# OpenNLPLab/ACR_WSSS

Hardware: AMD Instinct MI355X
Metric: img/s ACR-ViT-hybrid-base 448x448 train step (higher is better)
Workload: dtype f32_split; 1 GPU; BASELINE configs[1]: ViT-hybrid-base (DPT) 448x448, batch 16 per GPU, ACR train step (2 views, fwd+bwd+SGD); global_batch=16, classes=20, alpha=125, parallelism=dp1

## Files before the change

### acr_wsss_amd/_lib.py

```python
import ctypes
import os

import torch

_HERE = os.path.dirname(os.path.abspath(__file__))
LIB_PATH = os.environ.get("ACR_LIB_PATH") or os.path.join(_HERE, "libacr_hip.so")

ACR_F32, ACR_BF16, ACR_BF16_F32MATH, ACR_F32_BF16X3 = 0, 1, 2, 3
MATH = {"f32": 0, "f32_split": 1, "f32_fp16x2": 2}
BF16_F32MATH = False
GETAM_FUNCS = {"grad": 0, "cam_grad": 1, "grad_s": 2, "cam_grad_s": 3}

c_void_p, c_int32, c_int64, c_float, c_size_t = (ctypes.c_void_p, ctypes.c_int32, ctypes.c_int64,
                                                  ctypes.c_float, ctypes.c_size_t)


class AttnDesc(ctypes.Structure):
    _fields_ = [("B", c_int32), ("H", c_int32), ("T", c_int32), ("head_dim", c_int32),
                ("dtype", c_int32), ("scale", c_float),
                ("qkv_sb", c_int64), ("qkv_st", c_int64), ("qkv_sh", c_int64),
                ("o_sb", c_int64), ("o_st", c_int64), ("o_sh", c_int64)]


_P = ctypes.POINTER(AttnDesc)
# ... 3 lines not shown
    "acr_set_option": (c_int32, [c_int32, c_int32]),
    "acr_get_option": (c_int32, [c_int32]),
    "acr_attn_fwd": (c_int32, [_P, c_void_p, c_void_p, c_void_p, c_void_p, c_void_p, c_void_p, c_int64, c_int64,
                               c_void_p]),
    "acr_attn_bwd": (c_int32, [_P, c_void_p, c_void_p, c_void_p, c_void_p, c_void_p, c_void_p, c_void_p, c_int64,
                               c_int64, c_void_p, c_void_p, c_void_p, c_void_p, c_void_p]),
    "acr_attn_scores_floats": (c_int64, [_P]),
    "acr_attn_fwd_scores": (c_int32, [_P, c_void_p, c_void_p, c_void_p, c_void_p, c_void_p, c_void_p, c_void_p, c_int64, c_int64,
                                      c_void_p]),
    "acr_attn_fwd_scores_oimg": (c_int32, [_P, c_void_p, c_void_p, c_void_p, c_void_p, c_void_p, c_void_p, c_void_p, c_int64, c_int64,
                                           c_void_p, c_void_p]),
    "acr_attn_fwd_oimg_offered": (c_int32, [_P]),
    "acr_attn_bwd_scores": (c_int32, [_P, c_void_p, c_void_p, c_void_p, c_void_p, c_void_p, c_void_p, c_void_p, c_void_p, c_int64,
                                      c_int64, c_void_p, c_void_p, c_void_p, c_void_p, c_void_p]),
    "acr_attn_bwd_ws_floats": (c_int64, [_P]),
    "acr_split3_bf16": (c_int32, [c_void_p, c_int64, c_int64, c_int64, c_void_p, c_int64, c_void_p]),
    "acr_attn_probs": (c_int32, [_P, c_void_p, c_void_p, c_void_p, c_void_p, c_void_p]),
    "acr_attn_dprobs": (c_int32, [_P, c_void_p, c_void_p, c_void_p, c_void_p]),
    "acr_consistency_ws_floats": (c_size_t, [c_int32, c_int32, c_int32]),
    "acr_consistency_fwd": (c_int32, [c_void_p, c_void_p, c_int64, c_int32, c_int32, c_int32, c_int32, c_void_p,
                                      c_void_p, c_void_p]),
    "acr_consistency_bwd": (c_int32, [c_void_p, c_void_p, c_int64, c_int32, c_int32, c_int32, c_int32, c_void_p,
                                      c_void_p, c_void_p, c_int64, c_int64, c_void_p]),
    "acr_linear_bf16": (c_int32, [c_void_p, c_int64, c_void_p, c_int64, c_void_p, c_void_p, c_int64, c_void_p, c_int64,
                                  c_int32, c_int32, c_int32, c_void_p]),
    "acr_gemm_f32_ws_floats": (c_size_t, [c_int32, c_int32, c_int32, c_int32, c_int32]),
    "acr_x3_image_floats": (c_size_t, [c_int32, c_int32]),
    "acr_x3_colsum_ws_floats": (c_size_t, [c_int32, c_int32]),
    "acr_x3_image": (c_int32, [c_void_p, c_int64, c_int32, c_int32, c_void_p, c_void_p, c_void_p, c_void_p]),
    "acr_x3_image_t": (c_int32, [c_void_p, c_int64, c_int32, c_int32, c_void_p, c_void_p]),
# ... 184 lines not shown
```

### acr_wsss_amd/csrc/attn_f32.h

```cpp
#pragma once
#include <hip/hip_runtime.h>
#include <stdint.h>

struct AttnGeom {
    int B, H, T;
    float scale;
    int64_t sb, st, sh;
    int64_t osb, ost, osh;
};

void acr_attn_fwd_f32_dma(const AttnGeom& g, const float* q, const float* k, const float* v, float* o, float* lse2, float* pmean,
                          int64_t pmean_sb, int64_t pmean_st, hipStream_t st);
void acr_attn_bwd_f32_dma(const AttnGeom& g, const float* q, const float* k, const float* v, const float* o, const float* d_o,
                          const float* lse2, const float* gm, int64_t gm_sb, int64_t gm_st, float* dq, float* dk, float* dv,
                          float* delta, hipStream_t st);

void acr_attn_fwd_f32_sres(const AttnGeom& g, const float* q, const float* k, const float* v, float* o, float* lse2, float* scores,
                           float* pmean, int64_t pmean_sb, int64_t pmean_st, hipStream_t st);
void acr_attn_bwd_f32_sres(const AttnGeom& g, const float* q, const float* k, const float* v, const float* o, const float* d_o,
                           const float* lse2, const float* scores, const float* gm, int64_t gm_sb, int64_t gm_st, float* dq,
                           float* dk, float* dv, float* delta, hipStream_t st);
void acr_attn_pmean_sres(const AttnGeom& g, const float* scores, const float* lse2, float* pmean, int64_t pmean_sb, int64_t pmean_st,
                         hipStream_t st);
void acr_attn_delta_sres(const AttnGeom& g, const float* scores, const float* o, const float* d_o, const float* lse2, const float* gm,
                         int64_t gm_sb, int64_t gm_st, float* delta, hipStream_t st);

int64_t acr_attn_x3_scores_floats(const AttnGeom& g);
int64_t acr_attn_x3_bwd_ws_floats(const AttnGeom& g);
bool acr_attn_x3_fwd_uses_split_tail(int T);
void acr_attn_fwd_f32_x3(const AttnGeom& g, const float* q, const float* k, const float* v, float* o, float* lse2, float* scores,
                         float* pmean, int64_t pmean_sb, int64_t pmean_st, hipStream_t st, char* oimg = nullptr);
void acr_attn_bwd_f32_x3(const AttnGeom& g, const float* q, const float* k, const float* v, const float* o, const float* d_o,
                         const float* lse2, const float* scores, const float* gm, int64_t gm_sb, int64_t gm_st, float* dq, float* dk,
                         float* dv, float* delta_ws, hipStream_t st);
```

### acr_wsss_amd/csrc/attn_f32.hip

```cpp
#include "acr_common.h"
#include "attn_f32.h"

#define LDP 68
#define TILE_FLOATS (32 * LDP)

template <typename T, int NTHREADS>
__device__ __forceinline__ void stage_tile(float* lds, const T* g, int64_t st, int row0, int Tn, int tid, float mul) {
#pragma unroll
    for (int i = 0; i < 512 / NTHREADS; ++i) {
        const int slot = tid + i * NTHREADS;
        const int row = slot >> 4, c4 = slot & 15;
        f32x4 v = acr_load4<T>(g + (int64_t)min(row0 + row, Tn - 1) * st + c4 * 4) * mul;
        const f32x4 z = {0.f, 0.f, 0.f, 0.f};
        *reinterpret_cast<f32x4*>(lds + row * LDP + c4 * 4) = (row0 + row < Tn) ? v : z;
    }
}

template <typename T>
__device__ __forceinline__ void load_rows(float (&reg)[32], const T* g, int64_t st, int row0, int Tn, int lane, float mul) {
    const int r = lane & 31, h = lane >> 5;
    const float okm = (row0 + r < Tn) ? mul : 0.f;
    const T* p = g + (int64_t)min(row0 + r, Tn - 1) * st + 32 * h;
#pragma unroll
    for (int i = 0; i < 8; ++i) {
// ... 602 lines not shown
                  "acr_attn_fwd_scores_oimg: pmean row pitch < T or batch stride < T*pitch");
    ACR_CHECK_ARG(d->o_sh == 64 && d->o_st == (int64_t)d->H * 64 && d->o_sb == (int64_t)d->T * d->o_st,
                  "acr_attn_fwd_scores_oimg: o must be the dense (B, T, H*64) activation (its image is that of the (B*T) x (H*64) matrix)");
    rc = check_x3(d, "acr_attn_fwd_scores_oimg");
    if (rc) return rc;
    acr_attn_fwd_f32_x3(geom(d), (const float*)q, (const float*)k, (const float*)v, (float*)o, lse2, scores, pmean, pmean_sb, pmean_st,
                        (hipStream_t)stream, reinterpret_cast<char*>(o_image));
    return acr_check_launch("acr_attn_fwd_scores_oimg");
}

extern "C" int acr_attn_fwd_oimg_offered(const acr_attn_desc* d) {
    if (!d || d->dtype != ACR_F32_BF16X3 || d->T <= 0) return 0;
    return acr_attn_x3_fwd_uses_split_tail(d->T) ? 0 : 1;
}

extern "C" int acr_attn_bwd_scores(const acr_attn_desc* d, const void* q, const void* k, const void* v, const void* o,
                                   const void* d_o, const float* lse2, const float* scores, const float* gmean, int64_t gmean_sb,
                                   int64_t gmean_st, void* dq, void* dk, void* dv, float* delta_ws, void* stream) {
    int rc = check_desc(d, "acr_attn_bwd_scores");
    if (rc) return rc;
    if (d->dtype != ACR_F32 && d->dtype != ACR_F32_BF16X3) {
        acr_set_error("acr_attn_bwd_scores: fp32 tensors only (the bf16 kernels recompute the logits)");
        return ACR_ERR_UNSUPPORTED;
    }
    ACR_CHECK_ARG(q && k && v && o && d_o && lse2 && scores && dq && dk && dv && delta_ws, "acr_attn_bwd_scores: null pointer");
    ACR_CHECK_ARG(aligned16(q) && aligned16(k) && aligned16(v) && aligned16(o) && aligned16(d_o) && aligned16(scores),
                  "acr_attn_bwd_scores: inputs must be 16-byte aligned");
    ACR_CHECK_ARG(!gmean || (gmean_st >= d->T && gmean_sb >= (int64_t)d->T * gmean_st),
                  "acr_attn_bwd_scores: gmean row pitch < T or batch stride < T*pitch");
    ACR_CHECK_ARG(!gmean || ((gmean_st & 3) == 0 && (gmean_sb & 3) == 0 && aligned16(gmean)),
                  "acr_attn_bwd_scores: gmean must be 16-byte aligned with pitch and batch stride multiples of 4 floats");
    if (d->dtype == ACR_F32_BF16X3) {
        rc = check_x3(d, "acr_attn_bwd_scores");
        if (rc) return rc;
        ACR_CHECK_ARG(aligned16(delta_ws) && aligned16(dq) && aligned16(dk) && aligned16(dv), "acr_attn_bwd_scores: delta_ws / dq / dk / dv must be 16-byte aligned");
        acr_attn_bwd_f32_x3(geom(d), (const float*)q, (const float*)k, (const float*)v, (const float*)o, (const float*)d_o, lse2, scores,
                            gmean, gmean_sb, gmean_st, (float*)dq, (float*)dk, (float*)dv, delta_ws, (hipStream_t)stream);
        return acr_check_launch("acr_attn_bwd_scores");
    }
    acr_attn_bwd_f32_sres(geom(d), (const float*)q, (const float*)k, (const float*)v, (const float*)o, (const float*)d_o, lse2,
                          scores, gmean, gmean_sb, gmean_st, (float*)dq, (float*)dk, (float*)dv, delta_ws, (hipStream_t)stream);
    return acr_check_launch("acr_attn_bwd_scores");
}

extern "C" int acr_attn_probs(const acr_attn_desc* d, const void* q, const void* k, const float* lse2, float* probs,
                              void* stream) {
    int rc = check_desc(d, "acr_attn_probs");
    if (rc) return rc;
    ACR_CHECK_ARG(q && k && lse2 && probs, "acr_attn_probs: null pointer");
    AttnGeom g = geom(d);
    const int nt = (d->T + 63) / 64;
    ACR_CHECK_ARG((int64_t)d->B * d->H * nt * nt < (1ll << 31), "acr_attn_probs: grid too large");
    const dim3 grid(d->B * d->H * nt * nt);
    const void* pp[2] = {q, k};
    if (d->dtype == ACR_F32)
        hipLaunchKernelGGL((attn_tile_qk_kernel<float, TQK_PROBS>), grid, dim3(256), 0, (hipStream_t)stream, g,
                           (const float*)q, (const float*)k, lse2, probs, (int64_t)0, (int64_t)0);
// ... 66 lines not shown
```

### acr_wsss_amd/csrc/attn_f32_sres_tails.h

```cpp
#pragma once
#include "acr_common.h"
#include "attn_f32.h"
#include "attn_f32_tiles.h"

#define SB_FLOATS 1024
#define SRES_LOAD_NT(p) __builtin_nontemporal_load(reinterpret_cast<const f32x4*>(p))
#define SRES_LOAD(p) (*reinterpret_cast<const f32x4*>(p))
#define SRES_STORE(p, v) __builtin_nontemporal_store(v, reinterpret_cast<f32x4*>(p))
#define SRES_LOAD_DQ(p) SRES_LOAD_NT(p)
#define SRES_DMA_AUX 0

__device__ __forceinline__ int64_t sres_block(const AttnGeom& g, int NB, int b, int hd, int qb, int kb) {
    return ((((int64_t)b * g.H + hd) * NB + qb) * NB + kb) * SB_FLOATS;
}

__device__ __forceinline__ void wave_wait_dma() { asm volatile("s_waitcnt vmcnt(0)" ::: "memory"); }
__device__ __forceinline__ void wave_wait_lds() { asm volatile("s_waitcnt lgkmcnt(0)" ::: "memory"); }

template <int NW>
__device__ __forceinline__ void attn_fwd_tail_body(float* smem, float* mlsh, const AttnGeom& g, const float* __restrict__ q,
                                                   const float* __restrict__ k, const float* __restrict__ v, float* __restrict__ o,
                                                   float* __restrict__ lse2, float* __restrict__ sres, int id) {
    const int NB = (g.T + 31) >> 5;
    const int hd = id % g.H, b = id / g.H;
// ... 159 lines not shown
        const float* pw = smem + w * DT_FLOATS;
#pragma unroll
        for (int e = 0; e < 16; ++e) { dq0[e] += pw[e * 64 + lane]; dq1[e] += pw[(16 + e) * 64 + lane]; }
    }
#pragma unroll
    for (int reg = 0; reg < 16; ++reg) {
        const int qq = q0 + acr_krow(reg, h);
        if (qq < g.T) {
            float* p = dq + base + (int64_t)qq * g.st;
            p[r] = dq0[reg] * g.scale;
            p[32 + r] = dq1[reg] * g.scale;
        }
    }
}

template <int NW>
__device__ __forceinline__ void attn_dkdv_tail_body(float* smem, float* ssm, const AttnGeom& g, const float* __restrict__ q,
                                                    const float* __restrict__ v, const float* __restrict__ d_o,
                                                    const float* __restrict__ lse2, const float* __restrict__ delta,
                                                    const float* __restrict__ sres, const float* __restrict__ gm, int64_t gm_sb,
                                                    int64_t gm_st, float* __restrict__ dk, float* __restrict__ dv, int id) {
    const int NB = (g.T + 31) >> 5;
    const int hd = id % g.H, b = id / g.H;
    const int tid = threadIdx.x, lane = tid & 63;
    const int wave = __builtin_amdgcn_readfirstlane(tid >> 6);
    const int r = lane & 31, h = lane >> 5;
    const int key0 = (NB - 1) * 32;
    const int64_t base = (int64_t)b * g.sb + (int64_t)hd * g.sh;
    const int64_t obase = (int64_t)b * g.osb + (int64_t)hd * g.osh;
    const float* qb = q + base;
    const float* dob = d_o + obase;
    const float* lrow = lse2 + ((int64_t)b * g.H + hd) * g.T;
    const float* drow = delta + ((int64_t)b * g.H + hd) * g.T;
    const float* scol = sres + sres_block(g, NB, b, hd, 0, NB - 1);
    const int64_t sstep = (int64_t)NB * SB_FLOATS;
    float* tl = smem + wave * DT_FLOATS;
// ... 42 lines not shown
                if (q0 + acr_krow(reg, h) >= g.T) s[reg] = -INFINITY;
        }
        f32x16 p, ds;
#pragma unroll
        for (int gq = 0; gq < 4; ++gq) {
            const f32x4 l4 = *reinterpret_cast<const f32x4*>(rcw + 8 * gq + 4 * h);
            const f32x4 d4 = *reinterpret_cast<const f32x4*>(rcw + 32 + 8 * gq + 4 * h);
#pragma unroll
            for (int e = 0; e < 4; ++e) {
                const int reg = 4 * gq + e;
                const float pv = __builtin_amdgcn_exp2f(s[reg] - l4[e]);
                p[reg] = pv;
                ds[reg] = pv * (dp[reg] + gv[reg] - d4[e]);
            }
        }
        accop_a_i<0, 0>(dv0, p, sm, lb);
        accop_a_i<0, 1>(dv1, p, sm, lb);
        wave_wait_lds();
        dma_tile32_one(tl, qb, g.st, q0, g.T, lane);
        wave_wait_dma();
        accop_a_i<0, 0>(dk0, ds, sm, lb);
        accop_a_i<0, 1>(dk1, ds, sm, lb);
        wave_wait_lds();
    }
    __syncthreads();
#pragma unroll
    for (int e = 0; e < 16; ++e) {
        tl[e * 64 + lane] = dk0[e]; tl[(16 + e) * 64 + lane] = dk1[e];
        sw[e * 64 + lane] = dv0[e]; sw[(16 + e) * 64 + lane] = dv1[e];
    }
// ... 27 lines not shown
```

### acr_wsss_amd/csrc/attn_f32_x3.hip

```cpp
#include <type_traits>

#include "acr_split.h"
#include "attn_f32.h"
#include "attn_f32_sres_tails.h"

typedef __bf16 bf16_t;
typedef __attribute__((address_space(3))) void* x3_lds_vp;
typedef const __attribute__((address_space(1))) void* x3_glb_vp;

#define X3_PLANE_B (32 * 64 * 2)
#define X3_TILE_B (3 * X3_PLANE_B)
#define X3_SLOT_B (2 * X3_TILE_B)
#define X3_SB_FLOATS 1024

#define X3_STORE_NT(p, v) __builtin_nontemporal_store(v, reinterpret_cast<f32x4*>(p))
#define X3_LOAD_NT(p) __builtin_nontemporal_load(reinterpret_cast<const f32x4*>(p))


template <int N>
__device__ __forceinline__ void x3_vmcnt() { asm volatile("s_waitcnt vmcnt(%0)" ::"n"(N) : "memory"); }
__device__ __forceinline__ void x3_wait_vm(int n) {
    if (n >= 9) x3_vmcnt<9>();
    else if (n >= 8) x3_vmcnt<8>();
    else if (n >= 7) x3_vmcnt<7>();
// ... 449 lines not shown
        if (k0 + 32 < g.T) step(k0 + 32, std::integral_constant<int, 1>{});
    }
    if (!live) return;
    const int64_t base = (int64_t)b * g.sb + (int64_t)hd * g.sh;
#pragma unroll
    for (int reg = 0; reg < 16; ++reg) {
        const int qq = q0 + acr_krow(reg, h);
        if (qq < g.T) {
            float* p = dq + base + (int64_t)qq * g.st;
            p[r] = dq0[reg] * g.scale;
            p[32 + r] = dq1[reg] * g.scale;
        }
    }
}

__device__ __forceinline__ void attn_dkdv_x3_body(char* smem, float* ssm, float* gsm, float* rcm, int bid, int nblk, bool tails,
                                                  const X3Geom& g,
                                                  const bf16_t* __restrict__ qp, const bf16_t* __restrict__ vp,
                                                  const bf16_t* __restrict__ dop, const float* __restrict__ lse2,
                                                  const float* __restrict__ delta, const float* __restrict__ sres,
                                                  const float* __restrict__ gm, int64_t gm_sb, int64_t gm_st, float* __restrict__ dk,
                                                  float* __restrict__ dv) {
    const int NB = (g.T + 31) >> 5, nkt = tails ? NB / X3_BW : (NB + X3_BW - 1) / X3_BW;
    int id = acr_xcd_remap(bid, nblk);
    const int ktile = id % nkt; id /= nkt;
    const int hd = id % g.H;
    const int b = id / g.H;
    const int tid = threadIdx.x, lane = tid & 63;
    const int wave = __builtin_amdgcn_readfirstlane(tid >> 6);
    const int r = lane & 31, h = lane >> 5;
    const int key0 = (ktile * X3_BW + wave) * 32;
    const bool live = key0 < g.T;
    const int64_t pbase = (int64_t)b * g.T * g.D + (int64_t)hd * 64;
    const int op = wave >> 2, pc = wave & 3;
    const bf16_t* tb = (op ? dop : qp) + pbase;
    char* tdst = smem + op * X3_TILE_B;
    const float* lrow = lse2 + ((int64_t)b * g.H + hd) * g.T;
// ... 39 lines not shown
    f32x16 dk0 = {0}, dk1 = {0}, dv0 = {0}, dv1 = {0};
    const X3Lane lb = x3_lane(lane, smem);
    const int doff = x3_dma_off(g.D, pc, lane);
    uint32_t tb4[4];
    {
        const int gk = r >> 3, hk = (r >> 2) & 1, ek = r & 3, mm = 2 * gk + hk;
#pragma unroll
        for (int j = 0; j < 4; ++j)
            tb4[j] = x3_lds_addr(ssm) + ((wave * 2 * X3_SB_FLOATS) + gk * 256 + 128 * hk + ek + 4 * ((j + 4 * h) ^ mm)) * 4;
    }
    const uint32_t gaddr = x3_lds_addr(gsm) + (wave * X3_SB_FLOATS + 4 * h * 32 + r) * 4;
    const uint32_t rcaddr = x3_lds_addr(rcw) + 16 * h;
    auto step = [&](int q0, auto slot_tag) {
        constexpr int SLOT = decltype(slot_tag)::value;
        constexpr int QOFF = SLOT * X3_SLOT_B, DOOFF = QOFF + X3_TILE_B;
        x3_barrier((q0 > 0 && live) ? 1 + (gb0 ? 4 : 0) + (q0 + 32 < g.T ? 4 : 0) : 0);
        auto dma_next = [&] {
            if (q0 + 64 <= g.T) x3_dma_tile_i(tdst + (SLOT ^ 1) * X3_SLOT_B, tb + (int64_t)(q0 + 32) * g.D, g.plane, doff, pc);
            else if (q0 + 32 < g.T) x3_dma_tile(tdst + (SLOT ^ 1) * X3_SLOT_B, tb, g.plane, g.D, q0 + 32, g.T, pc, lane);
            X3_FENCE();
        };
        if (!live) { dma_next(); return; }
        f32x16 dp = {0};
        x3_rowop<DOOFF>(dp, lb, vf, dma_next);
        if (q0 > 0) x3_wait_vm(q0 + 32 < g.T ? 7 : 0);
        float s[16], gv[16];
        f32x4 l4[4], d4[4];
#define X3_RDS(REG) IMG_RD32(s[REG], tb4[(REG) & 3], SLOT * X3_SB_FLOATS * 4 + 128 * ((REG) >> 2))
#define X3_RDG(REG) IMG_RD32(gv[REG], gaddr, 128 * (((REG) & 3) + 8 * ((REG) >> 2)))
        X3_RDS(0); X3_RDS(1); X3_RDS(2); X3_RDS(3); X3_RDS(4); X3_RDS(5); X3_RDS(6); X3_RDS(7);
        X3_RDS(8); X3_RDS(9); X3_RDS(10); X3_RDS(11); X3_RDS(12); X3_RDS(13); X3_RDS(14); X3_RDS(15);
// ... 17 lines not shown
#pragma unroll
            for (int reg = 0; reg < 16; ++reg)
                if (q0 + acr_krow(reg, h) >= g.T) s[reg] = -INFINITY;
        }
        f32x16 p, ds;
#pragma unroll
        for (int gq = 0; gq < 4; ++gq) {
#pragma unroll
            for (int e = 0; e < 4; ++e) {
                const int reg = 4 * gq + e;
                const float pv = __builtin_amdgcn_exp2f(s[reg] - l4[gq][e]);
                p[reg] = pv;
                ds[reg] = pv * (dp[reg] + gv[reg] * invH - d4[gq][e]);
            }
        }
        asm volatile("s_waitcnt lgkmcnt(0)" ::: "memory");
        bf16x8 z0[3], z1[3];
        split3_bf16_acc<0>(p, z0);
        x3_accop<DOOFF, true>(dv0, dv1, z0, z1, lb,
                              [&] { split3_bf16_acc<1>(p, z1); },
                              [&] { if (q0 + 32 < g.T) dma_rc(q0 + 32); X3_FENCE(); },
                              [&] { if (q0 + 32 < g.T) dma_g(q0 + 32); X3_FENCE(); });
        split3_bf16_acc<0>(ds, z0);
        x3_accop<QOFF, true>(dk0, dk1, z0, z1, lb,
                             [&] { split3_bf16_acc<1>(ds, z1); },
                             [&] { if (q0 + 64 < g.T) dma_scores((q0 >> 5) + 2, SLOT); X3_FENCE(); });
    };
    for (int q0 = 0; q0 < g.T; q0 += 64) {
        step(q0, std::integral_constant<int, 0>{});
        if (q0 + 32 < g.T) step(q0 + 32, std::integral_constant<int, 1>{});
// ... 19 lines not shown
                                                                   const float* __restrict__ lse2, const float* __restrict__ delta,
                                                                   const float* __restrict__ sres, const float* __restrict__ gm,
                                                                   int64_t gm_sb, int64_t gm_st, float* __restrict__ dq,
                                                                   float* __restrict__ dk, float* __restrict__ dv,
                                                                   const float* __restrict__ q32, const float* __restrict__ k32,
                                                                   const float* __restrict__ v32, const float* __restrict__ do32,
                                                                   AttnGeom g32, int ntail) {
    __shared__ __attribute__((aligned(1024))) char lds[2 * X3_SLOT_B + X3_BW * 3 * X3_SB_FLOATS * 4 + X3_BW * 256];
    char* smem = lds;
    float* ssm = reinterpret_cast<float*>(lds + 2 * X3_SLOT_B);
    float* gsm = ssm + X3_BW * 2 * X3_SB_FLOATS;
    float* rcm = gsm + X3_BW * X3_SB_FLOATS;
    const int half = ((int)gridDim.x - 2 * ntail) >> 1;
    const int bid = (int)blockIdx.x;
    if (bid < half)
        attn_dkdv_x3_body(smem, ssm, gsm, rcm, bid, half, ntail != 0, g, qp, vp, dop, lse2, delta, sres, gm, gm_sb, gm_st, dk, dv);
    else if (bid < 2 * half)
        attn_dq_x3_body(smem, ssm, gsm, bid - half, half, ntail != 0, g, kp, vp, dop, lse2, delta, sres, gm, gm_sb, gm_st, dq);
    else if (bid < 2 * half + ntail)
        attn_dkdv_tail_body<X3_BW>(reinterpret_cast<float*>(lds), reinterpret_cast<float*>(lds) + X3_BW * DT_FLOATS, g32, q32, v32, do32, lse2,
                                   delta, sres, gm, gm_sb, gm_st, dk, dv, acr_xcd_remap(bid - 2 * half, ntail));
    else
        attn_dq_tail_body<X3_BW>(reinterpret_cast<float*>(lds), g32, k32, v32, do32, lse2, delta, sres, gm, gm_sb, gm_st, dq,
                                 acr_xcd_remap(bid - 2 * half - ntail, ntail));
}

static int64_t x3_score_floats(const AttnGeom& g) {
    const int64_t nb = (g.T + 31) / 32;
    return (int64_t)g.B * g.H * nb * nb * X3_SB_FLOATS;
}
int64_t acr_attn_x3_scores_floats(const AttnGeom& g) {
    return x3_score_floats(g) + 9 * ((int64_t)g.B * g.T * g.H * 64) / 2;
}
int64_t acr_attn_x3_bwd_ws_floats(const AttnGeom& g) {
    return (((int64_t)g.B * g.H * g.T + 3) & ~(int64_t)3) + 3 * ((int64_t)g.B * g.T * g.H * 64) / 2;
}
static bool x3_split_tail(int NB, int nw) { return (NB % nw) == 1 && NB > nw; }
static X3Geom x3_geom(const AttnGeom& g) {
    X3Geom x;
    x.B = g.B; x.H = g.H; x.T = g.T; x.D = g.H * 64; x.scale = g.scale;
    x.plane = (int64_t)g.B * g.T * x.D;
    x.osb = g.osb; x.ost = g.ost; x.osh = g.osh;
    x.sb = g.sb; x.st = g.st; x.sh = g.sh;
    return x;
}

bool acr_attn_x3_fwd_uses_split_tail(int T) {
    const int NB = (T + 31) / 32;
    return x3_split_tail(NB, 4) && NB >= 33;
}

// ... 3 lines not shown
    bf16_t* planes = reinterpret_cast<bf16_t*>(scores + x3_score_floats(g));
    X3SplitArgs a;
    a.src[0] = q; a.src[1] = k; a.src[2] = v;
    a.sb = g.sb; a.st = g.st; a.sh = g.sh; a.dst = planes; a.plane = x.plane; a.B = g.B; a.T = g.T; a.H = g.H;
    const int64_t n8 = (int64_t)g.B * g.T * g.H * 8;
    hipLaunchKernelGGL(x3_split_kernel, dim3((unsigned)((n8 + 255) / 256), 3), dim3(256), 0, st, a);
    const int NB = (g.T + 31) / 32;
    const int ntail = (acr_attn_x3_fwd_uses_split_tail(g.T) && oimg == nullptr) ? g.B * g.H : 0;
    hipLaunchKernelGGL(attn_fwd_x3_kernel, dim3(g.B * g.H * (ntail ? NB / 4 : (NB + 3) / 4) + ntail), dim3(256), 0, st, x, (const bf16_t*)planes,
                       (const bf16_t*)(planes + 3 * x.plane), (const bf16_t*)(planes + 6 * x.plane), o, lse2, scores, q, k, v, g, ntail, oimg);
    if (pmean) acr_attn_pmean_sres(g, scores, lse2, pmean, pmean_sb, pmean_st, st);
}

void acr_attn_bwd_f32_x3(const AttnGeom& g, const float* q, const float* k, const float* v, const float* o, const float* d_o,
                         const float* lse2, const float* scores, const float* gm, int64_t gm_sb, int64_t gm_st, float* dq, float* dk,
                         float* dv, float* delta_ws, hipStream_t st) {
    const X3Geom x = x3_geom(g);
    const bf16_t* planes = reinterpret_cast<const bf16_t*>(scores + x3_score_floats(g));
    bf16_t* dop = reinterpret_cast<bf16_t*>(delta_ws + (((int64_t)g.B * g.H * g.T + 3) & ~(int64_t)3));
    X3SplitArgs a;
    a.src[0] = d_o; a.src[1] = a.src[2] = nullptr;
    a.sb = g.osb; a.st = g.ost; a.sh = g.osh; a.dst = dop; a.plane = x.plane; a.B = g.B; a.T = g.T; a.H = g.H;
    const int64_t n8 = (int64_t)g.B * g.T * g.H * 8;
    hipLaunchKernelGGL(x3_split_kernel, dim3((unsigned)((n8 + 255) / 256), 1), dim3(256), 0, st, a);
    acr_attn_delta_sres(g, scores, o, d_o, lse2, gm, gm_sb, gm_st, delta_ws, st);
    const int NB = (g.T + 31) / 32;
    const int ntail = x3_split_tail(NB, X3_BW) ? g.B * g.H : 0;
    const int nmain = g.B * g.H * (ntail ? NB / X3_BW : (NB + X3_BW - 1) / X3_BW);
    hipLaunchKernelGGL(attn_bwd_x3_kernel, dim3(2 * nmain + 2 * ntail), dim3(64 * X3_BW), 0, st, x, planes, planes + 3 * x.plane,
                       planes + 6 * x.plane, (const bf16_t*)dop, lse2, (const float*)delta_ws, scores, gm, gm_sb, gm_st, dq, dk, dv, q, k, v, d_o, g,
                       ntail);
}

extern "C" int acr_split3_bf16(const float* x, int64_t rows, int64_t cols, int64_t ld, void* planes, int64_t plane_stride, void* stream) {
    ACR_CHECK_ARG(x && planes, "acr_split3_bf16: null pointer");
    ACR_CHECK_ARG(rows > 0 && cols > 0 && (cols % 8) == 0 && (ld % 4) == 0 && ld >= cols, "acr_split3_bf16: need cols %% 8 == 0, ld %% 4 == 0, ld >= cols");
    ACR_CHECK_ARG(plane_stride >= rows * cols && (plane_stride % 8) == 0, "acr_split3_bf16: plane stride must cover rows * cols and be a multiple of 8");
    ACR_CHECK_ARG(((uintptr_t)x & 15) == 0 && ((uintptr_t)planes & 15) == 0, "acr_split3_bf16: 16-byte alignment");
    const int64_t n = rows * (cols >> 3);
    ACR_CHECK_ARG((n + 255) / 256 < (1ll << 31), "acr_split3_bf16: too large");
    hipLaunchKernelGGL(x3_split2d_kernel, dim3((unsigned)((n + 255) / 256)), dim3(256), 0, (hipStream_t)stream, x, rows, cols, ld,
                       (bf16_t*)planes, plane_stride);
    return acr_check_launch("acr_split3_bf16");
}
```

### acr_wsss_amd/ops.py

```python
import os
import torch
from torch.autograd import Function

from . import _lib as L

HEAD_DIM = 64
ATTN_F32_SCORES = True


def pad4(n):
    return (n + 3) & ~3


def _desc(B, H, T, dtype, packed_qkv=True, math=0):
    D = H * HEAD_DIM
    d = L.AttnDesc()
    d.B, d.H, d.T, d.head_dim = B, H, T, HEAD_DIM
    d.dtype = L.ACR_F32_BF16X3 if (math == 1 and dtype == torch.float32) else L.dtype_code(dtype)
    d.scale = HEAD_DIM ** -0.5
    d.qkv_sb, d.qkv_st, d.qkv_sh = T * 3 * D, 3 * D, HEAD_DIM
    d.o_sb, d.o_st, d.o_sh = T * D, D, HEAD_DIM
    return d


# ... 126 lines not shown
        gm_sb = gm_st = 0
        if g_pm is not None:
            ok = (g_pm.dtype == torch.float32 and g_pm.stride(2) == 1 and g_pm.stride(1) % 4 == 0
                  and g_pm.stride(1) >= pad4(T) and g_pm.stride(0) % 4 == 0 and g_pm.data_ptr() % 16 == 0)
            if not ok:
                buf = torch.zeros((B, T, pad4(T)), dtype=torch.float32, device=qkv.device)
                buf[:, :, :T].copy_(g_pm)
                g_pm = buf[:, :, :T]
            gm_sb, gm_st = g_pm.stride(0), g_pm.stride(1)
        d = _desc(B, heads, T, qkv.dtype, math=ctx.math if scores is not None else 0)
        dqkv = torch.empty_like(qkv)
        delta = torch.empty(lib.acr_attn_bwd_ws_floats(d) if scores is not None else B * heads * T, dtype=torch.float32, device=qkv.device)
        qp, kp, vp = _qkv_ptrs(qkv, heads)
        dqp, dkp, dvp = _qkv_ptrs(dqkv, heads)
        tok = _t0("attn_bwd" if g_pm is not None else "attn_bwd_nomean", B, heads, T)
        if scores is not None:
            L.check(lib.acr_attn_bwd_scores(d, qp, kp, vp, L.ptr(o), L.ptr(d_o), L.ptr(lse2), L.ptr(scores), L.ptr(g_pm), gm_sb,
                                            gm_st, dqp, dkp, dvp, L.ptr(delta), L.stream_ptr()), "acr_attn_bwd_scores")
        else:
            L.check(lib.acr_attn_bwd(d, qp, kp, vp, L.ptr(o), L.ptr(d_o), L.ptr(lse2), L.ptr(g_pm), gm_sb, gm_st,
                                     dqp, dkp, dvp, L.ptr(delta), L.stream_ptr()), "acr_attn_bwd")
        _t1(tok)
        if ctx.owner is not None:
            ctx.owner._saved_do = d_o
            ctx.owner._saved_gpm = g_pm
        return dqkv, None, None, None, None, None, None


class StackAliasFn(Function):

    @staticmethod
# ... 1318 lines not shown
```

### include/acr_hip.h

```cpp
#ifndef ACR_HIP_H
#define ACR_HIP_H

#include <stddef.h>
#include <stdint.h>

#ifdef __cplusplus
extern "C" {
#endif

#define ACR_ABI_VERSION 2

typedef enum acr_status {
    ACR_OK = 0,
    ACR_ERR_INVALID = -1,
    ACR_ERR_LAUNCH = -2,
    ACR_ERR_UNSUPPORTED = -3
} acr_status;

typedef enum acr_dtype { ACR_F32 = 0, ACR_BF16 = 1, ACR_BF16_F32MATH = 2, ACR_F32_BF16X3 = 3 } acr_dtype;

typedef enum acr_math { ACR_MATH_F32 = 0, ACR_MATH_BF16X3 = 1, ACR_MATH_FP16X2 = 2 } acr_math;
#define ACR_FP16X2_REL 2.384185791015625e-07
#define ACR_FP16X2_FLOOR 1.8189894035458565e-12

// ... 27 lines not shown
                 void* dq, void* dk, void* dv, float* delta_ws, void* stream);

int64_t acr_attn_scores_floats(const acr_attn_desc* desc);
int64_t acr_attn_bwd_ws_floats(const acr_attn_desc* desc);
int acr_split3_bf16(const float* x, int64_t rows, int64_t cols, int64_t ld, void* planes, int64_t plane_stride, void* stream);
int acr_attn_fwd_scores(const acr_attn_desc* desc, const void* q, const void* k, const void* v,
                        void* o, float* lse2, float* scores, float* pmean, int64_t pmean_sb, int64_t pmean_st, void* stream);
int acr_attn_fwd_scores_oimg(const acr_attn_desc* desc, const void* q, const void* k, const void* v,
                             void* o, float* lse2, float* scores, float* pmean, int64_t pmean_sb, int64_t pmean_st, float* o_image,
                             void* stream);
int acr_attn_fwd_oimg_offered(const acr_attn_desc* desc);
int acr_attn_bwd_scores(const acr_attn_desc* desc, const void* q, const void* k, const void* v,
                        const void* o, const void* d_o, const float* lse2, const float* scores,
                        const float* gmean, int64_t gmean_sb, int64_t gmean_st,
                        void* dq, void* dk, void* dv, float* delta_ws, void* stream);

int acr_attn_probs(const acr_attn_desc* desc, const void* q, const void* k, const float* lse2,
                   float* probs, void* stream);
int acr_attn_dprobs(const acr_attn_desc* desc, const void* d_o, const void* v,
                    float* dprobs, void* stream);

int acr_linear_bf16(const void* a, int64_t lda, const void* b, int64_t ldb, const void* bias,
                    const void* resid, int64_t ldr, void* y, int64_t ldy, int32_t M, int32_t N, int32_t K,
                    void* stream);
int acr_linear_gelu_bf16(const void* a, int64_t lda, const void* w, int64_t ldw, const void* bias, void* h, void* act,
                         int64_t ldy, int32_t M, int32_t N, int32_t K, void* stream);
int acr_linear_dgelu_bf16(const void* a, int64_t lda, const void* w, int64_t ldw, const void* h, int64_t ldh, void* y,
                          int64_t ldy, int32_t M, int32_t N, int32_t K, void* stream);


// ... 213 lines not shown
```

Baseline: 127.3 img/s.

## Split x3 attention backward into dK/dV pass that stores dS, then dQ from dS

In the bf16x3 backward path, the fused kernel is replaced by two kernels. The first computes dK/dV and writes dS to a global workspace. The second reads dS back and computes dQ with a single GEMM against K, instead of recomputing P, dP and dS inside the dQ blocks. This removes the duplicated softmax-gradient recomputation. In exchange it costs a large extra f32 workspace the size of the scores buffer, extra HBM write and read traffic, and a second kernel launch that is serialized after the first.

```diff
diff --git a/acr_wsss_amd/_lib.py b/acr_wsss_amd/_lib.py
--- a/acr_wsss_amd/_lib.py
+++ b/acr_wsss_amd/_lib.py
@@ -41,6 +41,9 @@
     "acr_attn_bwd_scores": (c_int32, [_P, c_void_p, c_void_p, c_void_p, c_void_p, c_void_p, c_void_p, c_void_p, c_void_p, c_int64,
                                       c_int64, c_void_p, c_void_p, c_void_p, c_void_p, c_void_p]),
     "acr_attn_bwd_ws_floats": (c_int64, [_P]),
+    "acr_attn_bwd_ds_floats": (c_int64, [_P]),
+    "acr_attn_bwd_scores_ds": (c_int32, [_P, c_void_p, c_void_p, c_void_p, c_void_p, c_void_p, c_void_p, c_void_p, c_void_p, c_int64,
+                                         c_int64, c_void_p, c_void_p, c_void_p, c_void_p, c_void_p, c_void_p]),
     "acr_split3_bf16": (c_int32, [c_void_p, c_int64, c_int64, c_int64, c_void_p, c_int64, c_void_p]),
     "acr_attn_probs": (c_int32, [_P, c_void_p, c_void_p, c_void_p, c_void_p, c_void_p]),
     "acr_attn_dprobs": (c_int32, [_P, c_void_p, c_void_p, c_void_p, c_void_p]),
diff --git a/acr_wsss_amd/csrc/attn_f32.h b/acr_wsss_amd/csrc/attn_f32.h
--- a/acr_wsss_amd/csrc/attn_f32.h
+++ b/acr_wsss_amd/csrc/attn_f32.h
@@ -27,9 +27,10 @@
 
 int64_t acr_attn_x3_scores_floats(const AttnGeom& g);
 int64_t acr_attn_x3_bwd_ws_floats(const AttnGeom& g);
+int64_t acr_attn_x3_bwd_ds_floats(const AttnGeom& g);
 bool acr_attn_x3_fwd_uses_split_tail(int T);
 void acr_attn_fwd_f32_x3(const AttnGeom& g, const float* q, const float* k, const float* v, float* o, float* lse2, float* scores,
                          float* pmean, int64_t pmean_sb, int64_t pmean_st, hipStream_t st, char* oimg = nullptr);
 void acr_attn_bwd_f32_x3(const AttnGeom& g, const float* q, const float* k, const float* v, const float* o, const float* d_o,
                          const float* lse2, const float* scores, const float* gm, int64_t gm_sb, int64_t gm_st, float* dq, float* dk,
-                         float* dv, float* delta_ws, hipStream_t st);
+                         float* dv, float* delta_ws, float* ds, hipStream_t st);
diff --git a/acr_wsss_amd/csrc/attn_f32.hip b/acr_wsss_amd/csrc/attn_f32.hip
--- a/acr_wsss_amd/csrc/attn_f32.hip
+++ b/acr_wsss_amd/csrc/attn_f32.hip
@@ -640,9 +640,14 @@
     return acr_attn_x3_fwd_uses_split_tail(d->T) ? 0 : 1;
 }
 
-extern "C" int acr_attn_bwd_scores(const acr_attn_desc* d, const void* q, const void* k, const void* v, const void* o,
-                                   const void* d_o, const float* lse2, const float* scores, const float* gmean, int64_t gmean_sb,
-                                   int64_t gmean_st, void* dq, void* dk, void* dv, float* delta_ws, void* stream) {
+extern "C" int64_t acr_attn_bwd_ds_floats(const acr_attn_desc* d) {
+    if (d == nullptr || d->B <= 0 || d->H <= 0 || d->T <= 0 || d->dtype != ACR_F32_BF16X3) return 0;
+    return acr_attn_x3_bwd_ds_floats(geom(d));
+}
+
+static int attn_bwd_scores(const acr_attn_desc* d, const void* q, const void* k, const void* v, const void* o,
+                           const void* d_o, const float* lse2, const float* scores, const float* gmean, int64_t gmean_sb,
+                           int64_t gmean_st, void* dq, void* dk, void* dv, float* delta_ws, float* ds_ws, void* stream) {
     int rc = check_desc(d, "acr_attn_bwd_scores");
     if (rc) return rc;
     if (d->dtype != ACR_F32 && d->dtype != ACR_F32_BF16X3) {
@@ -661,12 +666,29 @@
         if (rc) return rc;
         ACR_CHECK_ARG(aligned16(delta_ws) && aligned16(dq) && aligned16(dk) && aligned16(dv), "acr_attn_bwd_scores: delta_ws / dq / dk / dv must be 16-byte aligned");
         acr_attn_bwd_f32_x3(geom(d), (const float*)q, (const float*)k, (const float*)v, (const float*)o, (const float*)d_o, lse2, scores,
-                            gmean, gmean_sb, gmean_st, (float*)dq, (float*)dk, (float*)dv, delta_ws, (hipStream_t)stream);
+                            gmean, gmean_sb, gmean_st, (float*)dq, (float*)dk, (float*)dv, delta_ws, ds_ws, (hipStream_t)stream);
         return acr_check_launch("acr_attn_bwd_scores");
     }
     acr_attn_bwd_f32_sres(geom(d), (const float*)q, (const float*)k, (const float*)v, (const float*)o, (const float*)d_o, lse2,
                           scores, gmean, gmean_sb, gmean_st, (float*)dq, (float*)dk, (float*)dv, delta_ws, (hipStream_t)stream);
     return acr_check_launch("acr_attn_bwd_scores");
+}
+
+extern "C" int acr_attn_bwd_scores(const acr_attn_desc* d, const void* q, const void* k, const void* v, const void* o,
+                                   const void* d_o, const float* lse2, const float* scores, const float* gmean, int64_t gmean_sb,
+                                   int64_t gmean_st, void* dq, void* dk, void* dv, float* delta_ws, void* stream) {
+    return attn_bwd_scores(d, q, k, v, o, d_o, lse2, scores, gmean, gmean_sb, gmean_st, dq, dk, dv, delta_ws, nullptr, stream);
+}
+
+extern "C" int acr_attn_bwd_scores_ds(const acr_attn_desc* d, const void* q, const void* k, const void* v, const void* o,
+                                      const void* d_o, const float* lse2, const float* scores, const float* gmean, int64_t gmean_sb,
+                                      int64_t gmean_st, void* dq, void* dk, void* dv, float* delta_ws, float* ds_ws, void* stream) {
+    if (d == nullptr || d->dtype != ACR_F32_BF16X3) {
+        acr_set_error("acr_attn_bwd_scores_ds: ACR_F32_BF16X3 only (the other arithmetics have no dS workspace)");
+        return ACR_ERR_UNSUPPORTED;
+    }
+    ACR_CHECK_ARG(ds_ws && aligned16(ds_ws), "acr_attn_bwd_scores_ds: ds_ws must be a 16-byte aligned buffer of acr_attn_bwd_ds_floats floats");
+    return attn_bwd_scores(d, q, k, v, o, d_o, lse2, scores, gmean, gmean_sb, gmean_st, dq, dk, dv, delta_ws, ds_ws, stream);
 }
 
 extern "C" int acr_attn_probs(const acr_attn_desc* d, const void* q, const void* k, const float* lse2, float* probs,
diff --git a/acr_wsss_amd/csrc/attn_f32_sres_tails.h b/acr_wsss_amd/csrc/attn_f32_sres_tails.h
--- a/acr_wsss_amd/csrc/attn_f32_sres_tails.h
+++ b/acr_wsss_amd/csrc/attn_f32_sres_tails.h
@@ -197,12 +197,13 @@
     }
 }
 
-template <int NW>
+template <int NW, bool DS = false>
 __device__ __forceinline__ void attn_dkdv_tail_body(float* smem, float* ssm, const AttnGeom& g, const float* __restrict__ q,
                                                     const float* __restrict__ v, const float* __restrict__ d_o,
                                                     const float* __restrict__ lse2, const float* __restrict__ delta,
                                                     const float* __restrict__ sres, const float* __restrict__ gm, int64_t gm_sb,
-                                                    int64_t gm_st, float* __restrict__ dk, float* __restrict__ dv, int id) {
+                                                    int64_t gm_st, float* __restrict__ dk, float* __restrict__ dv, int id,
+                                                    float* __restrict__ dsw = nullptr) {
     const int NB = (g.T + 31) >> 5;
     const int hd = id % g.H, b = id / g.H;
     const int tid = threadIdx.x, lane = tid & 63;
@@ -275,6 +276,16 @@
                 ds[reg] = pv * (dp[reg] + gv[reg] - d4[e]);
             }
         }
+        if constexpr (DS) {
+            float* dblk = dsw + sres_block(g, NB, b, hd, qt, NB - 1) + lane * 4;
+#pragma unroll
+            for (int gq = 0; gq < 4; ++gq) {
+                f32x4 t;
+#pragma unroll
+                for (int e = 0; e < 4; ++e) t[e] = (key < g.T && q0 + acr_krow(4 * gq + e, h) < g.T) ? ds[4 * gq + e] : 0.f;
+                SRES_STORE(dblk + gq * 256, t);
+            }
+        }
         accop_a_i<0, 0>(dv0, p, sm, lb);
         accop_a_i<0, 1>(dv1, p, sm, lb);
         wave_wait_lds();
diff --git a/acr_wsss_amd/csrc/attn_f32_x3.hip b/acr_wsss_amd/csrc/attn_f32_x3.hip
--- a/acr_wsss_amd/csrc/attn_f32_x3.hip
+++ b/acr_wsss_amd/csrc/attn_f32_x3.hip
@@ -487,13 +487,100 @@
     }
 }
 
+__device__ __forceinline__ void attn_dq_ds_x3_body(char* smem, float* ssm, int bid, int nblk, bool tails, const X3Geom& g,
+                                                   const bf16_t* __restrict__ kp, const float* __restrict__ dsr, float* __restrict__ dq) {
+    const int NB = (g.T + 31) >> 5, nqt = tails ? NB / X3_BW : (NB + X3_BW - 1) / X3_BW;
+    int id = acr_xcd_remap(bid, nblk);
+    const int qt = id % nqt; id /= nqt;
+    const int hd = id % g.H;
+    const int b = id / g.H;
+    const int tid = threadIdx.x, lane = tid & 63;
+    const int wave = __builtin_amdgcn_readfirstlane(tid >> 6);
+    const int r = lane & 31, h = lane >> 5;
+    const int q0 = (qt * X3_BW + wave) * 32;
+    const bool live = q0 < g.T;
+    const int pc = wave & 3;
+    const int plo = wave < 4 ? 0 : 2, phi = wave < 4 ? 2 : 3;
+    const int trow = 8 * pc + (lane >> 3);
+    const bf16_t* tb = kp + (int64_t)b * g.T * g.D + (int64_t)hd * 64 + (((lane & 7) ^ x3_swz(trow)) << 3);
+    auto dma_tile = [&](char* dst, int row0) {
+        const bf16_t* src = tb + (int64_t)min(row0 + trow, g.T - 1) * g.D;
+        for (int p = plo; p < phi; ++p)
+            __builtin_amdgcn_global_load_lds((x3_glb_vp)(src + p * g.plane), (x3_lds_vp)(dst + p * X3_PLANE_B + pc * 1024), 16, 0, 0);
+    };
+    const float* drow = dsr + x3_block(g.H, NB, b, hd, min(q0 >> 5, NB - 1), 0);
+    int soff[4];
+#pragma unroll
+    for (int gq = 0; gq < 4; ++gq) soff[gq] = gq * 256 + 4 * (lane ^ (2 * gq + (lane >> 5)));
+    float* sw = ssm + wave * 2 * X3_SB_FLOATS;
+    auto dma_ds = [&](int kblk, int slot) {
+        const float* src = drow + (int64_t)kblk * X3_SB_FLOATS;
+#pragma unroll
+        for (int gq = 0; gq < 4; ++gq)
+            __builtin_amdgcn_global_load_lds((x3_glb_vp)(src + soff[gq]), (x3_lds_vp)(sw + slot * X3_SB_FLOATS + gq * 256), 16, 0, 0);
+    };
+    dma_tile(smem, 0);
+    if (live) {
+        dma_ds(0, 0);
+        if (32 < g.T) dma_ds(1, 1);
+    }
+    f32x16 dq0 = {0}, dq1 = {0};
+    const X3Lane lb = x3_lane(lane, smem);
+    uint32_t tb4[4];
+    {
+        const int gk = r >> 3, hk = (r >> 2) & 1, ek = r & 3, mm = 2 * gk + hk;
+#pragma unroll
+        for (int j = 0; j < 4; ++j)
+            tb4[j] = x3_lds_addr(ssm) + ((wave * 2 * X3_SB_FLOATS) + gk * 256 + 128 * hk + ek + 4 * ((j + 4 * h) ^ mm)) * 4;
+    }
+    auto step = [&](int k0, auto slot_tag) {
+        constexpr int SLOT = decltype(slot_tag)::value;
+        constexpr int KOFF = SLOT * X3_TILE_B;
+        x3_barrier((k0 > 0 && live && k0 + 32 < g.T) ? 4 : 0);
+        if (k0 + 32 < g.T) dma_tile(smem + (SLOT ^ 1) * X3_TILE_B, k0 + 32);
+        X3_FENCE();
+        if (!live) return;
+        float s[16];
+#define X3_RDS(REG) IMG_RD32(s[REG], tb4[(REG) & 3], SLOT * X3_SB_FLOATS * 4 + 128 * ((REG) >> 2))
+        X3_RDS(0); X3_RDS(1); X3_RDS(2); X3_RDS(3); X3_RDS(4); X3_RDS(5); X3_RDS(6); X3_RDS(7);
+        X3_RDS(8); X3_RDS(9); X3_RDS(10); X3_RDS(11); X3_RDS(12); X3_RDS(13); X3_RDS(14); X3_RDS(15);
+#undef X3_RDS
+        asm volatile("s_waitcnt lgkmcnt(0)" : "+v"(s[0]), "+v"(s[1]), "+v"(s[2]), "+v"(s[3]), "+v"(s[4]), "+v"(s[5]), "+v"(s[6]), "+v"(s[7]),
+                     "+v"(s[8]), "+v"(s[9]), "+v"(s[10]), "+v"(s[11]), "+v"(s[12]), "+v"(s[13]), "+v"(s[14]), "+v"(s[15]) : : "memory");
+        f32x16 ds;
+#pragma unroll
+        for (int reg = 0; reg < 16; ++reg) ds[reg] = s[reg];
+        bf16x8 z0[3], z1[3];
+        split3_bf16_acc<0>(ds, z0);
+        x3_accop<KOFF, true>(dq0, dq1, z0, z1, lb,
+                             [&] { split3_bf16_acc<1>(ds, z1); },
+                             [&] { if (k0 + 64 < g.T) dma_ds((k0 >> 5) + 2, SLOT); X3_FENCE(); });
+    };
+    for (int k0 = 0; k0 < g.T; k0 += 64) {
+        step(k0, std::integral_constant<int, 0>{});
+        if (k0 + 32 < g.T) step(k0 + 32, std::integral_constant<int, 1>{});
+    }
+    if (!live) return;
+    const int64_t base = (int64_t)b * g.sb + (int64_t)hd * g.sh;
+#pragma unroll
+    for (int reg = 0; reg < 16; ++reg) {
+        const int qq = q0 + acr_krow(reg, h);
+        if (qq < g.T) {
+            float* p = dq + base + (int64_t)qq * g.st;
+            p[r] = dq0[reg] * g.scale;
+            p[32 + r] = dq1[reg] * g.scale;
+        }
+    }
+}
+
+template <bool DS>
 __device__ __forceinline__ void attn_dkdv_x3_body(char* smem, float* ssm, float* gsm, float* rcm, int bid, int nblk, bool tails,
                                                   const X3Geom& g,
                                                   const bf16_t* __restrict__ qp, const bf16_t* __restrict__ vp,
                                                   const bf16_t* __restrict__ dop, const float* __restrict__ lse2,
                                                   const float* __restrict__ delta, const float* __restrict__ sres,
                                                   const float* __restrict__ gm, int64_t gm_sb, int64_t gm_st, float* __restrict__ dk,
-                                                  float* __restrict__ dv) {
+                                                  float* __restrict__ dv, float* __restrict__ dsw) {
     const int NB = (g.T + 31) >> 5, nkt = tails ? NB / X3_BW : (NB + X3_BW - 1) / X3_BW;
     int id = acr_xcd_remap(bid, nblk);
     const int ktile = id % nkt; id /= nkt;
@@ -563,7 +650,13 @@
     auto step = [&](int q0, auto slot_tag) {
         constexpr int SLOT = decltype(slot_tag)::value;
         constexpr int QOFF = SLOT * X3_SLOT_B, DOOFF = QOFF + X3_TILE_B;
-        x3_barrier((q0 > 0 && live) ? 1 + (gb0 ? 4 : 0) + (q0 + 32 < g.T ? 4 : 0) : 0);
+        if constexpr (DS) {
+            const int nyoung = (q0 > 0 && live) ? 5 + (gb0 ? 4 : 0) + (q0 + 32 < g.T ? 4 : 0) : 0;
+            if (nyoung >= 13) { x3_vmcnt<13>(); acr_barrier_nofence(); }
+            else x3_barrier(nyoung);
+        } else {
+            x3_barrier((q0 > 0 && live) ? 1 + (gb0 ? 4 : 0) + (q0 + 32 < g.T ? 4 : 0) : 0);
+        }
         auto dma_next = [&] {
             if (q0 + 64 <= g.T) x3_dma_tile_i(tdst + (SLOT ^ 1) * X3_SLOT_B, tb + (int64_t)(q0 + 32) * g.D, g.plane, doff, pc);
             else if (q0 + 32 < g.T) x3_dma_tile(tdst + (SLOT ^ 1) * X3_SLOT_B, tb, g.plane, g.D, q0 + 32, g.T, pc, lane);
@@ -611,6 +704,20 @@
                 ds[reg] = pv * (dp[reg] + gv[reg] * invH - d4[gq][e]);
             }
         }
+        if constexpr (DS) {
+            if (q0 + 32 > g.T || key0 + 32 > g.T) {
+#pragma unroll
+                for (int reg = 0; reg < 16; ++reg)
+                    if (q0 + acr_krow(reg, h) >= g.T || key0 + r >= g.T) ds[reg] = 0.f;
+            }
+            float* dblk = dsw + (scol - sres) + (int64_t)(q0 >> 5) * sstep;
+#pragma unroll
+            for (int gq = 0; gq < 4; ++gq) {
+                const f32x4 t = {ds[4 * gq], ds[4 * gq + 1], ds[4 * gq + 2], ds[4 * gq + 3]};
+                X3_STORE_NT(dblk + gq * 256 + (unsigned)(lane * 4), t);
+            }
+            X3_FENCE();
+        }
         asm volatile("s_waitcnt lgkmcnt(0)" ::: "memory");
         bf16x8 z0[3], z1[3];
         split3_bf16_acc<0>(p, z0);
@@ -660,7 +767,7 @@
     const int half = ((int)gridDim.x - 2 * ntail) >> 1;
     const int bid = (int)blockIdx.x;
     if (bid < half)
-        attn_dkdv_x3_body(smem, ssm, gsm, rcm, bid, half, ntail != 0, g, qp, vp, dop, lse2, delta, sres, gm, gm_sb, gm_st, dk, dv);
+        attn_dkdv_x3_body<false>(smem, ssm, gsm, rcm, bid, half, ntail != 0, g, qp, vp, dop, lse2, delta, sres, gm, gm_sb, gm_st, dk, dv, nullptr);
     else if (bid < 2 * half)
         attn_dq_x3_body(smem, ssm, gsm, bid - half, half, ntail != 0, g, kp, vp, dop, lse2, delta, sres, gm, gm_sb, gm_st, dq);
     else if (bid < 2 * half + ntail)
@@ -671,6 +778,44 @@
                                  acr_xcd_remap(bid - 2 * half - ntail, ntail));
 }
 
+__global__ __launch_bounds__(64 * X3_BW, 2) void attn_dkdv_x3_kernel(X3Geom g, const bf16_t* __restrict__ qp, const bf16_t* __restrict__ vp,
+                                                                    const bf16_t* __restrict__ dop, const float* __restrict__ lse2,
+                                                                    const float* __restrict__ delta, const float* __restrict__ sres,
+                                                                    const float* __restrict__ gm, int64_t gm_sb, int64_t gm_st,
+                                                                    float* __restrict__ dk, float* __restrict__ dv, float* __restrict__ dsw,
+                                                                    const float* __restrict__ q32, const float* __restrict__ v32,
+                                                                    const float* __restrict__ do32, AttnGeom g32, int ntail) {
+    __shared__ __attribute__((aligned(1024))) char lds[2 * X3_SLOT_B + X3_BW * 3 * X3_SB_FLOATS * 4 + X3_BW * 256];
+    char* smem = lds;
+    float* ssm = reinterpret_cast<float*>(lds + 2 * X3_SLOT_B);
+    float* gsm = ssm + X3_BW * 2 * X3_SB_FLOATS;
+    float* rcm = gsm + X3_BW * X3_SB_FLOATS;
+    const int nmain = (int)gridDim.x - ntail;
+    const int bid = (int)blockIdx.x;
+    if (bid < nmain)
+        attn_dkdv_x3_body<true>(smem, ssm, gsm, rcm, bid, nmain, ntail != 0, g, qp, vp, dop, lse2, delta, sres, gm, gm_sb, gm_st, dk, dv, dsw);
+    else
+        attn_dkdv_tail_body<X3_BW, true>(reinterpret_cast<float*>(lds), reinterpret_cast<float*>(lds) + X3_BW * DT_FLOATS, g32, q32, v32, do32,
+                                         lse2, delta, sres, gm, gm_sb, gm_st, dk, dv, acr_xcd_remap(bid - nmain, ntail), dsw);
+}
+
+__global__ __launch_bounds__(64 * X3_BW, 2) void attn_dq_ds_x3_kernel(X3Geom g, const bf16_t* __restrict__ kp, const float* __restrict__ dsr,
+                                                                  const float* __restrict__ lse2, const float* __restrict__ delta,
+                                                                  const float* __restrict__ sres, const float* __restrict__ gm,
+                                                                  int64_t gm_sb, int64_t gm_st, float* __restrict__ dq,
+                                                                  const float* __restrict__ k32, const float* __restrict__ v32,
+                                                                  const float* __restrict__ do32, AttnGeom g32, int ntail) {
+    __shared__ __attribute__((aligned(1024))) char lds[2 * X3_TILE_B + X3_BW * 2 * X3_SB_FLOATS * 4];
+    static_assert(sizeof(lds) >= X3_BW * DT_FLOATS * 4, "the dQ split tail needs one tile image per wave");
+    const int nmain = (int)gridDim.x - ntail;
+    const int bid = (int)blockIdx.x;
+    if (bid < nmain)
+        attn_dq_ds_x3_body(lds, reinterpret_cast<float*>(lds + 2 * X3_TILE_B), bid, nmain, ntail != 0, g, kp, dsr, dq);
+    else
+        attn_dq_tail_body<X3_BW>(reinterpret_cast<float*>(lds), g32, k32, v32, do32, lse2, delta, sres, gm, gm_sb, gm_st, dq,
+                                 acr_xcd_remap(bid - nmain, ntail));
+}
+
 static int64_t x3_score_floats(const AttnGeom& g) {
     const int64_t nb = (g.T + 31) / 32;
     return (int64_t)g.B * g.H * nb * nb * X3_SB_FLOATS;
@@ -681,6 +826,7 @@
 int64_t acr_attn_x3_bwd_ws_floats(const AttnGeom& g) {
     return (((int64_t)g.B * g.H * g.T + 3) & ~(int64_t)3) + 3 * ((int64_t)g.B * g.T * g.H * 64) / 2;
 }
+int64_t acr_attn_x3_bwd_ds_floats(const AttnGeom& g) { return x3_score_floats(g); }
 static bool x3_split_tail(int NB, int nw) { return (NB % nw) == 1 && NB > nw; }
 static X3Geom x3_geom(const AttnGeom& g) {
     X3Geom x;
@@ -714,7 +860,7 @@
 
 void acr_attn_bwd_f32_x3(const AttnGeom& g, const float* q, const float* k, const float* v, const float* o, const float* d_o,
                          const float* lse2, const float* scores, const float* gm, int64_t gm_sb, int64_t gm_st, float* dq, float* dk,
-                         float* dv, float* delta_ws, hipStream_t st) {
+                         float* dv, float* delta_ws, float* ds, hipStream_t st) {
     const X3Geom x = x3_geom(g);
     const bf16_t* planes = reinterpret_cast<const bf16_t*>(scores + x3_score_floats(g));
     bf16_t* dop = reinterpret_cast<bf16_t*>(delta_ws + (((int64_t)g.B * g.H * g.T + 3) & ~(int64_t)3));
@@ -727,9 +873,16 @@
     const int NB = (g.T + 31) / 32;
     const int ntail = x3_split_tail(NB, X3_BW) ? g.B * g.H : 0;
     const int nmain = g.B * g.H * (ntail ? NB / X3_BW : (NB + X3_BW - 1) / X3_BW);
-    hipLaunchKernelGGL(attn_bwd_x3_kernel, dim3(2 * nmain + 2 * ntail), dim3(64 * X3_BW), 0, st, x, planes, planes + 3 * x.plane,
-                       planes + 6 * x.plane, (const bf16_t*)dop, lse2, (const float*)delta_ws, scores, gm, gm_sb, gm_st, dq, dk, dv, q, k, v, d_o, g,
-                       ntail);
+    if (ds == nullptr) {
+        hipLaunchKernelGGL(attn_bwd_x3_kernel, dim3(2 * nmain + 2 * ntail), dim3(64 * X3_BW), 0, st, x, planes, planes + 3 * x.plane,
+                           planes + 6 * x.plane, (const bf16_t*)dop, lse2, (const float*)delta_ws, scores, gm, gm_sb, gm_st, dq, dk, dv, q, k, v, d_o, g,
+                           ntail);
+        return;
+    }
+    hipLaunchKernelGGL(attn_dkdv_x3_kernel, dim3(nmain + ntail), dim3(64 * X3_BW), 0, st, x, planes, planes + 6 * x.plane, (const bf16_t*)dop, lse2,
+                       (const float*)delta_ws, scores, gm, gm_sb, gm_st, dk, dv, ds, q, v, d_o, g, ntail);
+    hipLaunchKernelGGL(attn_dq_ds_x3_kernel, dim3(nmain + ntail), dim3(64 * X3_BW), 0, st, x, planes + 3 * x.plane, (const float*)ds, lse2,
+                       (const float*)delta_ws, scores, gm, gm_sb, gm_st, dq, k, v, d_o, g, ntail);
 }
 
 extern "C" int acr_split3_bf16(const float* x, int64_t rows, int64_t cols, int64_t ld, void* planes, int64_t plane_stride, void* stream) {
diff --git a/acr_wsss_amd/ops.py b/acr_wsss_amd/ops.py
--- a/acr_wsss_amd/ops.py
+++ b/acr_wsss_amd/ops.py
@@ -164,7 +164,11 @@
         qp, kp, vp = _qkv_ptrs(qkv, heads)
         dqp, dkp, dvp = _qkv_ptrs(dqkv, heads)
         tok = _t0("attn_bwd" if g_pm is not None else "attn_bwd_nomean", B, heads, T)
-        if scores is not None:
+        if scores is not None and ctx.math == 1:
+            ds = torch.empty(lib.acr_attn_bwd_ds_floats(d), dtype=torch.float32, device=qkv.device)
+            L.check(lib.acr_attn_bwd_scores_ds(d, qp, kp, vp, L.ptr(o), L.ptr(d_o), L.ptr(lse2), L.ptr(scores), L.ptr(g_pm), gm_sb,
+                                               gm_st, dqp, dkp, dvp, L.ptr(delta), L.ptr(ds), L.stream_ptr()), "acr_attn_bwd_scores_ds")
+        elif scores is not None:
             L.check(lib.acr_attn_bwd_scores(d, qp, kp, vp, L.ptr(o), L.ptr(d_o), L.ptr(lse2), L.ptr(scores), L.ptr(g_pm), gm_sb,
                                             gm_st, dqp, dkp, dvp, L.ptr(delta), L.stream_ptr()), "acr_attn_bwd_scores")
         else:
diff --git a/include/acr_hip.h b/include/acr_hip.h
--- a/include/acr_hip.h
+++ b/include/acr_hip.h
@@ -65,6 +65,11 @@
                         const void* o, const void* d_o, const float* lse2, const float* scores,
                         const float* gmean, int64_t gmean_sb, int64_t gmean_st,
                         void* dq, void* dk, void* dv, float* delta_ws, void* stream);
+int64_t acr_attn_bwd_ds_floats(const acr_attn_desc* desc);
+int acr_attn_bwd_scores_ds(const acr_attn_desc* desc, const void* q, const void* k, const void* v,
+                           const void* o, const void* d_o, const float* lse2, const float* scores,
+                           const float* gmean, int64_t gmean_sb, int64_t gmean_st,
+                           void* dq, void* dk, void* dv, float* delta_ws, float* ds_ws, void* stream);
 
 int acr_attn_probs(const acr_attn_desc* desc, const void* q, const void* k, const float* lse2,
                    float* probs, void* stream);
```

Measured after the change: 128.4 img/s (median of 6 runs). No clear change (+0.9%).
